# risc-mi/totalsegmentator2D

Hardware: AMD Instinct MI355X
Metric: 2-ch 512x512 slices/sec (higher is better)
Workload: dtype f32 storage/accumulate, products as 3x fp16-split MFMA (f16x3)

## Files before the change

### totalsegmentator2d_amd/csrc/dispatch.cpp

```cpp
#include "engine_internal.h"
#include "tile_dims.h"

#include <algorithm>

namespace ts2d {

namespace {

inline int lg_exact(int v) { return (v > 0 && (v & (v - 1)) == 0) ? ilog2(v) : -1; }

inline void tile_finish(TileGeom& g, int B, int Ht, int Wt, int sy, int sx, int taps) {
    const bool p2 = lg_exact(g.TH) >= 0 && lg_exact(g.TW) >= 0;
    g.lgTH = p2 ? ilog2(g.TH) : -1; g.lgTW = p2 ? ilog2(g.TW) : -1;
    if (g.NIMG > 1) { g.tiles_x = 1; g.tiles_y = 1; }
    else { g.tiles_x = (Wt + g.TW - 1) / g.TW; g.tiles_y = (Ht + g.TH - 1) / g.TH; }
    g.n_mtiles = (B + g.NIMG - 1) / g.NIMG * g.tiles_x * g.tiles_y;
    const int halo = (taps == 9) ? 3 : 1;
    g.PH = (g.TH - 1) * sy + halo; g.PW = (g.TW - 1) * sx + halo;
}

TileGeom tile_geom_pow2(int B, int Ht, int Wt, int sy, int sx, int taps) {
    TileGeom g{};
    g.TW = std::min(32, pow2ceil(Wt));
    g.TH = std::min(pow2ceil(Ht), kBM / g.TW);
// ... 208 lines not shown
        if (ck != K_NONE) {
            c.k = ck; c.fused_stats = true;
            if (ck == K_UP0 && f16) c.ppt = 4;
            c.bn = op.cout % 64 == 0 ? 64 : 32;
            if (Ht % 8 || Wt % 32) { bool ok = false; c.g = tile_geom_upc(B, Ht, Wt, ok); c.flex = true; }
            else c.g = tile_fixed(B, Ht, Wt, (ck == K_UPQ || ck == K_UPC_H2) ? 16 : 8, 32, 1, 1);
            if (ck == K_UPC_H || ck == K_UPC_H2) c.ks = e->ops[op.up_idx].cin % 64 == 0 ? 4 : 2;
            if (ck == K_UP0) {
                c.seg = segment_tiles(e, c.g);
                if (e->u0seg > 0 && (c.g.tiles_x * c.g.tiles_y) % e->u0seg == 0) c.seg = e->u0seg;
            }
            return c;
        }
    }
    c.bn = op.cout % 64 == 0 ? 64 : 32;
    if (!(op.split_ok && !exact)) {
        if (f16 && op.stride != 3) return c;
        c.k = K_EXACT;
        c.g = tile_geom(B, Ht, Wt, op.sy, op.sx, 9);
        c.fused_stats = c.g.NIMG == 1;
        return c;
    }
    const bool img32 = fits32((size_t)Hin * Win * std::max(op.cin, op.cin_skip) * 4) && fits32((size_t)Ht * Wt * op.cout * 4);
    if (op.stride == 2) {
        int s2k = 1;
        {
            const TileGeom g1 = tile_geom(B, Ht, Wt, 2, 2, 9);
            const int P1 = g1.PH * g1.PW * g1.NIMG;
            if (e->use_one && g1.NIMG == 1 && P1 <= 5 * kBlock && img32) s2k = fill_ksplit(e, (long long)g1.n_mtiles * (op.cout / c.bn), op.cin / 8, full);
        }
        if (s2k == 1 && op.s2v2_ok && e->use_s2v2 && e->use_one && Ht % 8 == 0 && Wt % 32 == 0 && img32 && magic_ok(tile_fixed(B, Ht, Wt, 8, 32, 2, 2))) {
            c.k = K_S2_V2; c.bn = op.bn2; c.fused_stats = true;
            c.g = tile_fixed(B, Ht, Wt, 8, 32, 2, 2);
            s2v2_variant(e, op, c);
            return c;
        }
        if (s2k == 1 && op.s2v2_ok && e->use_s2v2 && e->use_one && e->use_flex2 && img32 && (f16 || e->use_flex2 > 1)) {
            bool ok = false;
            const TileGeom gs = tile_geom_s2v2(B, Ht, Wt, ok);
            if (ok && magic_ok(gs)) { c.k = K_S2_V2; c.bn = op.bn2; c.fused_stats = true; c.flex = true; c.g = gs; s2v2_variant(e, op, c); return c; }
        }
        c.g = tile_geom(B, Ht, Wt, 2, 2, 9);
        c.ksplit = std::max(choose_ksplit(op, c.g), s2k);
        c.fused_stats = c.g.NIMG == 1 && c.ksplit == 1;
        const int P = c.g.PH * c.g.PW * c.g.NIMG;
        c.k = (e->use_one && c.g.NIMG == 1 && P <= 5 * kBlock && img32) ? K_S2_ONE : K_S2_GENERIC;
        return c;
    }
    if (op.res_ok && e->use_res && e->use_one && src.normed && op.skip < 0 && Ht % 8 == 0 && Wt % 32 == 0 && fits32((size_t)Ht * Wt * 32 * 4)) {
        c.k = (oi == 1 && fuse0_applies(e, H, W)) ? K_S1_RES32F : K_S1_RES32;
        c.fused_stats = true;
        c.g = tile_fixed(B, Ht, Wt, 8, 32, 1, 1);
        c.seg = segment_tiles(e, c.g);
        return c;
    }
    c.g = tile_geom(B, Ht, Wt, 1, 1, 9);
    c.ksplit = choose_ksplit(op, c.g);
    c.fused_stats = c.g.NIMG == 1;
    const int P = c.g.PH * c.g.PW * c.g.NIMG;
    const bool srcs_normed = src.normed && (op.skip < 0 || e->tensors[op.skip].normed);
    const bool tiles16 = Ht % 16 == 0 && Wt % 32 == 0 && c.g.NIMG == 1 && img32;
    if (c.g.NIMG == 1 && img32 && op.cout % c.bn == 0) {
        const bool can = f16 ? (op.h32_ok && P * 4 <= 6 * kBlock) : (e->use_one && P * 2 <= 3 * kBlock);
        const int sk = can ? fill_ksplit(e, (long long)c.g.n_mtiles * (op.cout / c.bn), ct / (f16 ? 32 : 16), full) : 1;
        if (sk > 1) {
            c.ksplit = sk; c.fused_stats = false;
            c.k = f16 ? K_S1_H32 : K_S1_ONE;
            return c;
        }
    }
    if (f16) {
        if (e->use_h2 && tiles16 && op.cout % 64 == 0 && op.skip < 0 && ct % 32 == 0 && src.normed && ct >= kH2Min) {
            c.k = K_S1_H2; c.bn = 64;
            c.g = tile_fixed(B, Ht, Wt, 16, 32, 1, 1);
            return c;
        }
        c.k = (op.h32_ok && c.g.NIMG == 1 && P * 4 <= 6 * kBlock && img32) ? K_S1_H32 : K_S1_GENERIC;
        return c;
    }
    const bool one = e->use_one && c.g.NIMG == 1 && P * 2 <= 3 * kBlock && img32;
    if (one && e->use_q && tiles16 && c.bn == 64 && ct >= 64 && srcs_normed && magic_ok(tile_fixed(B, Ht, Wt, 16, 32, 1, 1))) {
        c.k = K_S1_QP;
        c.g = tile_fixed(B, Ht, Wt, 16, 32, 1, 1);
        return c;
    }
    c.k = one ? K_S1_ONE : K_S1_GENERIC;
    return c;
}

const char* kernel_name(const Op& op, const Choice& c) {
    const bool b64 = c.bn == 64;
    switch (c.k) {
    case K_NONE: case K_FUSED_AWAY: return "";
    case K_FIRST: return c.first_split ? "conv3x3_first_split" : "conv3x3_first";
    case K_FIRST_STATS: return "conv3x3_first_stats";
    case K_EXACT: return op.type == OP_CONV ? "conv_mfma_f32" : "convT_mfma_f32";
    case K_S1_GENERIC: return "conv3x3_f16x3";
    case K_S1_ONE: return b64 ? "conv3x3_f16x3_one<64>" : "conv3x3_f16x3_one<32>";
    case K_S1_QP: return "conv3x3_f16x3_qp";
    case K_S1_H32: return b64 ? "conv3x3_h32<64>" : "conv3x3_h32<32>";
    case K_S1_H2: return "conv3x3_h2";
    case K_S1_RES32: return "conv3x3_res32";
    case K_S1_RES32F: return "conv3x3_res32f";
    case K_S2_V2: return c.bn == 128 ? (c.k32 ? "conv3x3s2_v2<128,k32>" : "conv3x3s2_v2<128>") : (c.k32 ? "conv3x3s2_v2<64,k32>" : "conv3x3s2_v2<64>");
    case K_S2_ONE: return "conv3x3s2_f16x3_one";
    case K_S2_GENERIC: return "conv3x3s2_f16x3";
// ... 157 lines not shown
```

### totalsegmentator2d_amd/csrc/engine.hip

```cpp
#include "engine_internal.h"
#include "kernels.h"
#include "kernels_f16x3.h"
#include "kernels_f16x3_convt.h"
#include "kernels_h32.h"
#include "kernels_head.h"
#include "kernels_f16x3_one.h"
#include "kernels_f16x3_qp.h"
#include "kernels_first.h"
#include "kernels_res32.h"
#include "kernels_s2v2.h"
#include "kernels_upc.h"
#include "kernels_up0.h"
#include "kernels_upq.h"
#include "kernels_upc_h.h"
#include "kernels_upc_h2.h"
#include "kernels_resblock.h"

#include <atomic>
#include <cstdio>
#include <cmath>
#include <cstdlib>
#include <cstring>
#include <string>
#include <type_traits>
// ... 205 lines not shown
int launch_composed(ts2d_engine* e, size_t oi, const Choice& c, const Run& r) {
    if (c.k == K_UP0) return launch_up0(e, oi, c, r);
    const Op& op = e->ops[oi]; const Op& up = e->ops[op.up_idx];
    const Tensor& xc = e->tensors[up.src]; const Tensor& sk = e->tensors[op.skip];
    const TileGeom& g = c.g;
    const float* wts = e->d_weights;
    const int bn = c.bn;
    UpcArgs ua{};
    ua.xc = xc.data; ua.scc = xc.scale; ua.shc = xc.shift; ua.Cb = up.cin;
    ua.xs = sk.data; ua.scs = sk.scale; ua.shs = sk.shift; ua.Cs = op.cin_skip;
    ua.wc = wts + op.dev_wc; ua.wk = wts + op.dev_wk; ua.bvar = wts + op.dev_bvar; ua.oscale = wts + op.dev_wcs;
    ua.dst = e->tensors[op.dst].data; ua.part = e->d_part;
    ua.B = r.B; ua.H = r.H >> op.ly; ua.W = r.W >> op.lx; ua.Cout = op.cout;
    ua.tiles_x = g.tiles_x; ua.tiles_y = g.tiles_y; ua.n_mtiles = g.n_mtiles; ua.n_ctiles = op.cout / bn;
    ua.TH = g.TH; ua.TW = g.TW; ua.inv_twc = 1.0f / (float)(g.TW / 2);
    ua.slope = e->arch.leaky_slope;
    ua.prof = prof_slots(e, oi); ua.dbg = e->dbg;
    const dim3 grid((ua.n_mtiles + 7) / 8 * 8 * ua.n_ctiles), block(kBlock);
    const bool b64 = bn == 64, flex = c.flex;
    hipError_t launch;
    if (c.k == K_UPC_H2) {
        launch = c.ks == 4 ? launch_max_lds<conv3x3_upc_h2<4>>(grid, block, kUh2Lds, r.st, ua) : launch_max_lds<conv3x3_upc_h2<2>>(grid, block, kUh2Lds, r.st, ua);
    } else if (c.k == K_UPC_H) {
        const size_t smem = std::max((size_t)c.ks * 2 * kUcPlane, (size_t)4 * kUsPlane + (size_t)2 * 9 * 2 * bn * 16);
        auto inst = [&](auto bn_, auto ks_) {
            constexpr int BN = decltype(bn_)::value, KS = decltype(ks_)::value;
            return flex ? launch_max_lds<conv3x3_upc_h<BN, KS, true>>(grid, block, smem, r.st, ua) : launch_max_lds<conv3x3_upc_h<BN, KS>>(grid, block, smem, r.st, ua);
        };
        using I32 = std::integral_constant<int, 32>; using I64 = std::integral_constant<int, 64>;
        using K2 = std::integral_constant<int, 2>; using K4 = std::integral_constant<int, 4>;
        launch = b64 ? (c.ks == 4 ? inst(I64{}, K4{}) : inst(I64{}, K2{})) : (c.ks == 4 ? inst(I32{}, K4{}) : inst(I32{}, K2{}));
    } else if (c.k == K_UPQ) {
        launch = launch_max_lds<conv3x3_upq>(grid, dim3(kUqThreads), kUqLds, r.st, ua);
    } else {
        const size_t smem = std::max((size_t)8 * kUcPlane, (size_t)4 * kUsPlane + (size_t)9 * 4 * bn * 16);
        if (b64) launch = flex ? launch_max_lds<conv3x3_upc<64, true>>(grid, block, smem, r.st, ua) : launch_max_lds<conv3x3_upc<64, false>>(grid, block, smem, r.st, ua);
        else launch = flex ? launch_max_lds<conv3x3_upc<32, true>>(grid, block, smem, r.st, ua) : launch_max_lds<conv3x3_upc<32, false>>(grid, block, smem, r.st, ua);
    }
    HIP_TRY(launch);
    return TS2D_OK;
}

int launch_res32(ts2d_engine* e, size_t oi, const Choice& c, const Run& r) {
    const Op& op = e->ops[oi];
    const Tensor& src = e->tensors[op.src];
    const float* wts = e->d_weights;
    Res32Args ra{};
    ra.src = src.data; ra.sc = src.scale; ra.sh = src.shift; ra.wres = wts + op.dev_wres; ra.bias = wts + op.dev_b;
    ra.oscale = wts + op.dev_ws; ra.dst = e->tensors[op.dst].data; ra.part = e->d_part;
    ra.B = r.B; ra.H = r.H >> op.ly; ra.W = r.W >> op.lx; ra.tiles_x = c.g.tiles_x; ra.tiles_y = c.g.tiles_y; ra.n_tiles = c.g.n_mtiles;
    ra.slope = e->arch.leaky_slope;
    ra.prof = prof_slots(e, oi);
    ra.seg = c.seg;
    const bool fuse0 = c.k == K_S1_RES32F;
    if (fuse0) {
        if (!e->fused_away[0]) return fail(TS2D_ERR_INVALID, "internal: fused second block without the statistics-only first pass");
        const Op& o0 = e->ops[0];
        ra.src = nullptr; ra.x0 = r.d_in; ra.C0 = o0.cin; ra.w0 = wts + o0.dev_wraw; ra.b0 = wts + o0.dev_b;
    }
    const dim3 grid(ra.n_tiles / ra.seg), block(kBlock);
    const hipError_t launch = with_storage(r.f16, [&](auto s) {
        using S = decltype(s); using ST = typename S::type;
        const size_t smem = S::np == 3 ? 9 * 2 * 4 * 512 + 8 * kResPS : 9 * 4 * 512 + 4 * kResPS + 1536;
        return fuse0 ? launch_max_lds<conv3x3_res32<ST, S::np, true>>(grid, block, smem, r.st, ra) : launch_max_lds<conv3x3_res32<ST, S::np, false>>(grid, block, smem, r.st, ra);
    });
    HIP_TRY(launch);
    return TS2D_OK;
}

int launch_head(ts2d_engine* e, size_t oi, const Choice& c, const Run& r) {
    const Op& op = e->ops[oi];
    const Tensor& src = e->tensors[op.src];
    const float* wts = e->d_weights;
    HeadArgs ha{};
    ha.src = src.data; ha.sc = src.scale; ha.sh = src.shift; ha.w = wts + op.dev_w; ha.bias = wts + op.dev_b;
    ha.logits = r.d_logits; ha.mask = r.d_mask; ha.C = src.C; ha.K = op.cout; ha.HW = r.H * r.W;
    ha.total = (long long)r.B * r.H * r.W; ha.slope = e->arch.leaky_slope; ha.nonfinite = e->d_flags;
    if (c.k == K_HEAD_MFMA) {
        ha.wph = wts + op.dev_wh; ha.oscale = wts + op.dev_ws;
        const int bpw = 16;
        const long long nblk = ha.total / 32;
        const dim3 grid((unsigned)((nblk + 4 * bpw - 1) / (4 * bpw)));
        const hipError_t launch = with_storage(r.f16, [&](auto s) { using S = decltype(s); return launch_kernel<head_mfma32<typename S::type, S::np>>(grid, dim3(256), 0, r.st, ha, bpw); });
        HIP_TRY(launch);
        return TS2D_OK;
    }
    const dim3 grid((unsigned)((ha.total + 255) / 256));
    const size_t smem = ((size_t)256 * (src.C + 1) + (size_t)op.cout * src.C + op.cout) * sizeof(float);
    const hipError_t launch = with_storage(r.f16, [&](auto s) {
        using ST = typename decltype(s)::type;
        return src.C == 32 ? launch_max_lds<head_1x1<32, ST>>(grid, dim3(256), smem, r.st, ha) : launch_max_lds<head_1x1<64, ST>>(grid, dim3(256), smem, r.st, ha);
    });
    HIP_TRY(launch);
    return TS2D_OK;
}

int launch_proj(ts2d_engine* e, size_t oi, const Choice& c, const Run& r) {
    const Op& op = e->ops[oi];
    const Tensor& src = e->tensors[op.src];
    ProjArgs pa{};
    pa.src = src.data; pa.sc = src.scale; pa.sh = src.shift; pa.w = e->d_weights + op.dev_w; pa.dst = e->tensors[op.dst].data;
    pa.part = c.fused_stats ? e->d_part : nullptr;
    pa.Cin = src.C; pa.Cout = op.cout; pa.sy = op.sy; pa.sx = op.sx;
    pa.Wt = r.W >> op.lx; pa.HW = (r.H >> op.ly) * pa.Wt; pa.Win = r.W >> src.lx; pa.M = r.B * pa.HW;
    pa.slope = e->arch.leaky_slope; pa.inv_n = 1.0f / (float)(op.sy * op.sx);
    if (!src.normed || src.linear || src.C % 32 || op.cout % c.bn || (r.H >> src.ly) != (r.H >> op.ly) * op.sy || pa.Win != pa.Wt * op.sx)
// ... 356 lines not shown
    if (he != hipSuccess) {
        rc = fail(he == hipErrorOutOfMemory ? TS2D_ERR_NOMEM : TS2D_ERR_HIP, "engine setup failed: %s", hipGetErrorString(he));
        ts2d_engine_destroy(e);
        return rc;
    }
    if (weights) {
        rc = upload_weights(e, weights, n_floats);
        if (rc != TS2D_OK) { ts2d_engine_destroy(e); return rc; }
    }
    *out = e;
    return TS2D_OK;
}

int ts2d_engine_create(const ts2d_arch_desc* arch, const float* weights, size_t n_floats, int device, ts2d_engine** out) {
    return create_engine("ts2d_engine_create", arch, nullptr, weights, n_floats, device, out);
}

int ts2d_engine_create_residual(const ts2d_arch_desc* arch, const ts2d_residual_desc* residual, const float* weights, size_t n_floats, int device,
                                ts2d_engine** out) {
    if (!residual) return fail(TS2D_ERR_INVALID, "ts2d_engine_create_residual: null argument");
    return create_engine("ts2d_engine_create_residual", arch, residual, weights, n_floats, device, out);
}

int ts2d_engine_load_weights(ts2d_engine* e, const float* weights, size_t n_floats) {
    if (!e || !weights) return fail(TS2D_ERR_INVALID, "ts2d_engine_load_weights: null argument");
    HIP_TRY(hipSetDevice(e->device));
    if (e->ws_busy) { HIP_TRY(hipEventSynchronize(e->ws_event)); e->ws_busy = false; }
    HIP_TRY(hipStreamSynchronize(e->stream));
    return upload_weights(e, weights, n_floats);
}

int ts2d_engine_weight_buffer(ts2d_engine* e, void** dev_ptr, size_t* n_bytes) {
    if (!e || !dev_ptr || !n_bytes) return fail(TS2D_ERR_INVALID, "ts2d_engine_weight_buffer: null argument");
    *dev_ptr = e->d_weights; *n_bytes = e->weight_floats * sizeof(float);
    return TS2D_OK;
}

int ts2d_engine_set_precision(ts2d_engine* e, int mode) {
    if (!e) return fail(TS2D_ERR_INVALID, "ts2d_engine_set_precision: null engine");
    if (mode != TS2D_PRECISION_F32_EXACT && mode != TS2D_PRECISION_F32_SPLIT_F16X3 && mode != TS2D_PRECISION_F16)
        return fail(TS2D_ERR_INVALID, "unknown precision mode %d", mode);
    if (mode == TS2D_PRECISION_F16 && e->residual)
        return fail(TS2D_ERR_INVALID, "TS2D_PRECISION_F16 is not supported on a residual-encoder engine (TS2D_PRECISION_F32_SPLIT_F16X3 and "
                    "TS2D_PRECISION_F32_EXACT are); the mode is unchanged");
    e->precision = mode;
    return TS2D_OK;
}

int ts2d_engine_set_option(ts2d_engine* e, const char* name, int value) {
    if (!e || !name) return fail(TS2D_ERR_INVALID, "ts2d_engine_set_option: null argument");
    struct B { const char* n; bool* p; };
    struct I { const char* n; int* p; int lo, hi; };
    const B bools[] = {{"one", &e->use_one}, {"s2v2", &e->use_s2v2}, {"q", &e->use_q}, {"h2", &e->use_h2},  {"uh2", &e->use_uh2},
                       {"first_split", &e->use_first_split}, {"sbk", &e->use_sbk}, {"s2k32", &e->use_s2k32}, {"up0", &e->use_up0}, {"upc", &e->use_upc}, {"res", &e->use_res}, {"fuse0", &e->use_fuse0}, {"flex", &e->use_flex}};
    const I ints[] = {{"u0seg", &e->u0seg, 0, 1 << 20}, {"flex2", &e->use_flex2, 0, 2}};
    bool found = false;
    for (const B& b : bools) if (!strcmp(name, b.n)) { *b.p = value != 0; found = true; }
    for (const I& i : ints) if (!strcmp(name, i.n)) {
        if (value < i.lo || value > i.hi) return fail(TS2D_ERR_INVALID, "option %s = %d out of range [%d, %d]", name, value, i.lo, i.hi);
        *i.p = value; found = true;
    }
    if (!found) return fail(TS2D_ERR_INVALID, "unknown option '%s' (one s2v2 q h2 uh2 up0 u0seg upc res fuse0 flex flex2 first_split sbk s2k32)", name);
    e->ws_precision = -1;
    ++e->opt_gen;
    return TS2D_OK;
}

int ts2d_engine_set_keep_activations(ts2d_engine* e, int enable) {
    if (!e) return fail(TS2D_ERR_INVALID, "ts2d_engine_set_keep_activations: null engine");
    e->keep_activations = enable != 0;
    return TS2D_OK;
}

int ts2d_engine_set_tile_dtype(ts2d_engine* e, int mode) {
    if (!e) return fail(TS2D_ERR_INVALID, "ts2d_engine_set_tile_dtype: null engine");
    if (mode != TS2D_TILE_F32 && mode != TS2D_TILE_F16) return fail(TS2D_ERR_INVALID, "unknown tile dtype %d", mode);
    e->tile_half = mode == TS2D_TILE_F16;
    return TS2D_OK;
}

int ts2d_engine_weights_ready(ts2d_engine* e) {
    if (!e) return fail(TS2D_ERR_INVALID, "ts2d_engine_weights_ready: null engine");
    e->weights_ready = true;
    return TS2D_OK;
}

int ts2d_engine_reserve(ts2d_engine* e, int B, int H, int W) {
    if (!e) return fail(TS2D_ERR_INVALID, "ts2d_engine_reserve: null engine");
    return reserve_checked(e, B, H, W, kBySize);
}

int ts2d_engine_workspace_bytes(ts2d_engine* e, int B, int H, int W, size_t* n_bytes) {
    if (!e || !n_bytes) return fail(TS2D_ERR_INVALID, "ts2d_engine_workspace_bytes: null argument");
    const int divy = 1 << e->lvl_y[e->arch.n_stages - 1], divx = 1 << e->lvl_x[e->arch.n_stages - 1];
    if (B < 1 || H < divy || W < divx || H % divy || W % divx)
        return fail(TS2D_ERR_INVALID, "shape B=%d H=%d W=%d: H and W must be positive multiples of %d and %d", B, H, W, divy, divx);
    *n_bytes = workspace_layout(e, B, H, W, kBySize).bytes;
    return TS2D_OK;
}

int ts2d_engine_set_workspace(ts2d_engine* e, void* dev_ptr, size_t n_bytes) {
    if (!e) return fail(TS2D_ERR_INVALID, "ts2d_engine_set_workspace: null engine");
    if (dev_ptr && (reinterpret_cast<uintptr_t>(dev_ptr) & 255)) return fail(TS2D_ERR_INVALID, "ts2d_engine_set_workspace: the pointer must be 256-byte aligned");
    HIP_TRY(hipSetDevice(e->device));
    if (e->ws_busy) { HIP_TRY(hipEventSynchronize(e->ws_event)); e->ws_busy = false; }
    HIP_TRY(hipStreamSynchronize(e->stream));
    if (e->d_ws && !e->ws_external) HIP_TRY(hipFree(e->d_ws));
    e->d_ws = reinterpret_cast<char*>(dev_ptr); e->ws_bytes = dev_ptr ? n_bytes : 0; e->ws_external = dev_ptr != nullptr;
    e->ws_precision = -1; e->wsB = 0;
    for (Tensor& t : e->tensors) { t.data = nullptr; t.bytes = 0; t.resident = false; }
    e->lastB = 0;
    return TS2D_OK;
}

int ts2d_engine_forward(ts2d_engine* e, const float* input, int B, int H, int W, float* logits, uint32_t* mask_packed,
// ... 213 lines not shown
```

### totalsegmentator2d_amd/csrc/engine_internal.h

```cpp
#pragma once
#include "../../include/ts2d_engine.h"
#include <hip/hip_runtime_api.h>
#include "device_tables.h"

#include <atomic>
#include <cstddef>
#include <cstdint>
#include <string>
#include <vector>

#pragma GCC visibility push(hidden)
namespace ts2d {

int fail(int code, const char* fmt, ...) __attribute__((format(printf, 2, 3)));
const char* last_error();

#define HIP_TRY(expr)                                                                                     \
    do {                                                                                                  \
        hipError_t _e = (expr);                                                                           \
        if (_e != hipSuccess)                                                                             \
            return fail(_e == hipErrorOutOfMemory ? TS2D_ERR_NOMEM : TS2D_ERR_HIP, "%s failed: %s (%s:%d)", \
                        #expr, hipGetErrorString(_e), __FILE__, __LINE__);                                \
    } while (0)
#define TRY(expr) do { int _rc = (expr); if (_rc != TS2D_OK) return _rc; } while (0)
// ... 80 lines not shown
    int bn = 0;
    int ksplit = 1;
    bool fused_stats = false;
    int ppt = 1;
    bool first_full = false;
    bool flex = false;
    bool first_split = false;
    bool k32 = false;
    int npp = 0, nch = 0;
    int seg = 0;
    int ks = 0;
    const char* name = "";
};

inline int pow2ceil(int v) { int p = 1; while (p < v) p <<= 1; return p; }
inline int ilog2(int v) { int l = 0; while ((1 << l) < v) ++l; return l; }
inline int ct_total(const Op& op) { return op.cin + op.cin_skip; }

}

#pragma GCC visibility pop

struct ts2d_engine {
    ts2d_arch_desc arch{};
    int lvl_y[TS2D_MAX_STAGES] = {0}, lvl_x[TS2D_MAX_STAGES] = {0};
    int device = 0;
    int cin_pad = 8;
    std::vector<ts2d::Tensor> tensors;
    std::vector<ts2d::Op> ops;
    size_t blob_floats = 0;
    ts2d_arch_desc user_arch{};
    bool residual = false;
    int n_blocks[TS2D_MAX_STAGES] = {0};
    bool padded = false;
    size_t user_blob_floats = 0;
    float* d_weights = nullptr; size_t weight_floats = 0;
    bool weights_ready = false;
    int precision = TS2D_PRECISION_F32_SPLIT_F16X3;
    int num_cus = 256;
    int tile_half = 0;
    int tiled_inf = 0;
    bool use_one = true;
    bool use_s2v2 = true;
    bool use_q = true;
    bool use_h2 = true;
    bool use_uh2 = true;
    bool use_s2k32 = true;
    bool use_sbk = true;
    bool use_first_split = true;
    bool use_up0 = true;
    int u0seg = 0;
    bool use_upc = true;
    bool use_res = true;
    bool use_fuse0 = true;
    bool diagnosing = false;
    int use_flex2 = 2;
    bool use_flex = true;
    int dbg = 0;
    unsigned long long* d_prof = nullptr;
    std::vector<char> fused_away;
    char* d_ws = nullptr; size_t ws_bytes = 0; int wsB = 0, wsH = 0, wsW = 0;
    bool ws_external = false;
    uint32_t ws_token = 0;
    std::vector<ts2d::Choice> plan; int planB = 0, planH = 0, planW = 0, plan_prec = -1; unsigned plan_gen = 0, opt_gen = 1; bool plan_full = false;
    char* d_stage = nullptr; size_t stage_bytes = 0;
    bool ws_full = false;
    bool last_full = false;
    int ws_precision = -1; bool ws_keep = false;
    bool keep_activations = false;
    float* d_part = nullptr;
    float* d_partial = nullptr;
    float* d_up = nullptr;
    float* d_in_stage = nullptr; float* d_logit_stage = nullptr; uint32_t* d_mask_stage = nullptr;
    hipStream_t stream = nullptr;
    bool profiling = false;
    std::vector<ts2d::Launch> launches; size_t n_launched = 0;
    int lastB = 0, lastH = 0, lastW = 0; hipStream_t last_stream = nullptr; bool last_f16 = false;
    char* d_sw = nullptr; size_t sw_bytes = 0;
    hipEvent_t ws_event = nullptr; hipStream_t ws_stream = nullptr; bool ws_busy = false;
    int* d_flags = nullptr;
    bool checked_input = false; const float* last_input = nullptr;
};

#pragma GCC visibility push(hidden)
namespace ts2d {

ts2d_arch_desc pad_arch(const ts2d_arch_desc& a, bool& padded);
void expand_blob(const ts2d_arch_desc& ua, const ts2d_arch_desc& pa, const int* n_blocks, const float* ub, std::vector<float>& pb);
int build_program(ts2d_engine* e);
int tensor_index(ts2d_engine* e, const std::string& name);

void pack_weights(const ts2d_engine* e, const float* blob, float* out);
float f16_to_f32(uint16_t hb);

constexpr size_t kSbkElems = (size_t)2 * 256 * 256 * 64;
constexpr bool kBySize = false, kFullBatch = true;

Choice choose(const ts2d_engine* e, size_t oi, int B, int H, int W, bool full);
std::vector<Choice> choose_all(const ts2d_engine* e, int B, int H, int W, bool full);
const std::vector<Choice>& planned(ts2d_engine* e, int B, int H, int W, bool full);

struct ActPlan { std::vector<size_t> off, size; std::vector<char> used, reused; size_t bytes = 0; };
struct WsLayout {
    ActPlan plan; std::vector<size_t> o_sc, o_sh; size_t o_part = 0, o_pk = 0, o_up = 0, bytes = 0;
    bool has_up = false;
};
// ... 40 lines not shown
```

### totalsegmentator2d_amd/csrc/kernels_res32.h

```cpp
#pragma once
#include "kernels_f16x3.h"
#include "kernels_h32.h"

namespace ts2d {

struct Res32Args {
    const void* src; const float* sc; const float* sh;
    const void* wres;
    const float* bias;
    const float* oscale;
    void* dst;
    float* part;
    int B, H, W;
    int tiles_x, tiles_y;
    int n_tiles;
    int seg;
    float slope;
    unsigned long long* prof;
    const float* x0; int C0;
    const float* w0; const float* b0;
};

constexpr int kResPW = 34, kResP = 340, kResPS = 352 * 16;

template <typename ST, int NP, bool FUSE = false>
__global__ __launch_bounds__(kBlock, 2) void conv3x3_res32(const Res32Args a) {
    constexpr int NPP = NP == 3 ? 2 : 1;
    constexpr int WB = 9 * NPP * 4 * 512;
    constexpr int NL = sizeof(ST) == 4 ? 2 : 1;
    constexpr int NU = 6;
    extern __shared__ __attribute__((aligned(16))) unsigned char smem8[];
    typedef unsigned u32x4 __attribute__((ext_vector_type(4)));

    const int tid = threadIdx.x, lane = tid & 63;
    const int w = __builtin_amdgcn_readfirstlane(tid >> 6);
    const int r = lane & 31, h = lane >> 5;

    const int tpi = a.tiles_x * a.tiles_y;
    const int t0 = (int)blockIdx.x * a.seg;
    if (t0 >= a.n_tiles) return;
    const int t1 = t0 + a.seg;
    const int n = t0 / tpi;
    int trem = t0 - n * tpi;
    int txi = trem / a.tiles_y, tyi = trem - txi * a.tiles_y;

    {
        const uint4* wsrc = reinterpret_cast<const uint4*>(a.wres);
#pragma unroll
        for (int k = 0; k < (WB / 16 + kBlock - 1) / kBlock; ++k) {
            const int sl = tid + k * kBlock;
            if (sl < WB / 16) *reinterpret_cast<uint4*>(smem8 + sl * 16) = wsrc[NPP == 2 ? sl : (sl >> 7) * 256 + (sl & 127)];
        }
    }
    unsigned char* sP = smem8 + WB;
    const int sg = (lane >> 3) & 3, pl = (lane & 7) + 8 * (lane >> 5);
    auto scratch32 = [&](int ww, int half) -> float* {
        if (NPP == 2) return reinterpret_cast<float*>(sP + (2 * ww + half) * kResPS + kResP * 16);
        return reinterpret_cast<float*>(sP + NPP * 4 * kResPS + (ww * 2 + half) * 192);
    };
    unsigned rel[FUSE ? 1 : NU];
    unsigned emask = 0;
    bool last_unit = false;
    const int swr = sg * kResPS + (16 * w + pl) * 16;
    const size_t img_bytes = (size_t)a.H * a.W * 32 * sizeof(ST);
    u32x4 pv[FUSE ? 1 : NU][NL];
    const int r2 = lane & 31, h2 = lane >> 5;
    constexpr int NK = 3;
    unsigned xrel[FUSE ? NK : 1], pq[FUSE ? NK : 1];
    float xv[FUSE ? NK : 1][FUSE ? 9 : 1];
    float wr0[FUSE ? 9 : 1], scq[FUSE ? 16 : 1], shq[FUSE ? 16 : 1];
    float bq[(FUSE && sizeof(ST) != 4) ? 16 : 1];
    typedef unsigned u32x4w __attribute__((ext_vector_type(4)));
    u32x4w wsp[FUSE ? 4 : 1];
    float inv_s0 = 1.f;
    const bool have3 = w != 3;
    __amdgpu_buffer_rsrc_t rs, rsx;
    if constexpr (!FUSE) {
#pragma unroll
        for (int it = 0; it < NU; ++it) {
            const int p = 64 * it + 16 * w + pl;
            const int py = p / kResPW, px = p - py * kResPW;
            rel[it] = (unsigned)(((py * a.W + px) * 32 + 8 * sg) * (int)sizeof(ST));
            if (p < kResP) emask |= ((py == 0 ? 1u : 0u) | (py == 9 ? 2u : 0u) | (px == 0 ? 4u : 0u) | (px == kResPW - 1 ? 8u : 0u)) << (4 * it);
        }
        last_unit = 64 * (NU - 1) + 16 * w + pl < kResP;
        rs = __builtin_amdgcn_make_buffer_rsrc(const_cast<unsigned char*>(reinterpret_cast<const unsigned char*>(a.src)) + (size_t)n * img_bytes,
                                               0, (int)img_bytes, 0x00020000);
    } else {
#pragma unroll
        for (int k = 0; k < NK; ++k) {
            const int p = 32 * (w + 4 * k) + r2;
            const int py = p / kResPW, px = p - py * kResPW;
            xrel[k] = (unsigned)(((h2 * a.H + py) * a.W + px) * 4);
            pq[k] = (unsigned)((py << 8) | px);
            if (p < kResP) emask |= ((py == 0 ? 1u : 0u) | (py == 9 ? 2u : 0u) | (px == 0 ? 4u : 0u) | (px == kResPW - 1 ? 8u : 0u)) << (4 * k);
        }
        const size_t in_bytes = (size_t)a.C0 * a.H * a.W * 4;
        rsx = __builtin_amdgcn_make_buffer_rsrc(const_cast<float*>(a.x0) + (size_t)n * a.C0 * a.H * a.W, 0, (int)in_bytes, 0x00020000);
#pragma unroll
        for (int tap = 0; tap < 9; ++tap) wr0[tap] = h2 < a.C0 ? a.w0[((size_t)r2 * a.C0 + h2) * 9 + tap] : 0.f;
        {
            float wmax = 0.f;
#pragma unroll
            for (int tap = 0; tap < 9; ++tap) wmax = fmaxf(wmax, fabsf(wr0[tap]));
#pragma unroll
            for (int d = 1; d < 64; d *= 2) wmax = fmaxf(wmax, __shfl_xor(wmax, d));
            int e2 = 0;
            (void)frexpf(wmax, &e2);
            const bool sane = wmax > 0.f && wmax < 3.0e38f;
            const float S0 = sane ? ldexpf(1.f, 12 - e2) : 1.f;
            inv_s0 = sane ? ldexpf(1.f, e2 - 12) : 1.f;
            unsigned short wh[9], wl[9];
#pragma unroll
            for (int tap = 0; tap < 9; ++tap) {
                wr0[tap] *= S0;
                const _Float16 hh = (_Float16)wr0[tap], ll = (_Float16)(wr0[tap] - (float)hh);
                wh[tap] = __builtin_bit_cast(unsigned short, hh); wl[tap] = __builtin_bit_cast(unsigned short, ll);
            }
            auto pk = [](unsigned short lo_, unsigned short hi_) { return (unsigned)lo_ | ((unsigned)hi_ << 16); };
            wsp[0] = u32x4w{pk(wh[0], wh[1]), pk(wh[2], wh[3]), pk(wh[0], wh[1]), pk(wh[2], wh[3])};
            wsp[1] = u32x4w{pk(wh[4], wh[5]), pk(wh[6], wh[7]), pk(wh[4], wh[5]), pk(wh[6], wh[7])};
            wsp[2] = u32x4w{pk(wh[8], wh[8]), pk(wl[8], 0), 0u, 0u};
            wsp[3] = u32x4w{pk(wl[0], wl[1]), pk(wl[2], wl[3]), pk(wl[4], wl[5]), pk(wl[6], wl[7])};
        }
#pragma unroll
        for (int i = 0; i < 16; ++i) {
            const int c = (i & 3) + 8 * (i >> 2) + 4 * h2;
            const float s_ = a.sc[(size_t)n * 32 + c], t_ = a.sh[(size_t)n * 32 + c], b_ = a.b0[c];
            if constexpr (sizeof(ST) == 4) { scq[i] = s_ * inv_s0; shq[i] = __builtin_fmaf(b_, s_, t_); }
            else { scq[i] = s_; shq[i] = t_; bq[i] = b_; }
        }
    }
    auto prefetch = [&](int ptx, int pty) {
        if constexpr (!FUSE) {
            const unsigned org = (unsigned)((((pty * 8 - 1) * a.W + (ptx * 32 - 1)) * 32) * (int)sizeof(ST));
#pragma unroll
            for (int it = 0; it < NU; ++it)
#pragma unroll
                for (int l = 0; l < NL; ++l)
                    pv[it][l] = __builtin_amdgcn_raw_buffer_load_b128(rs, org + rel[it] + 16 * l, 0, 0);
        } else {
            const int oy0 = pty * 8 - 2, ox0 = ptx * 32 - 2;
            const bool pe = (pty == 0) | (pty == a.tiles_y - 1) | (ptx == 0) | (ptx == a.tiles_x - 1);
            const unsigned org = (unsigned)((oy0 * a.W + ox0) * 4);
#pragma unroll
            for (int k = 0; k < NK; ++k) {
                if (k < NK - 1 || have3) {
#pragma unroll
                    for (int tap = 0; tap < 9; ++tap) {
                        const int dy = tap / 3, dx = tap - 3 * dy;
                        unsigned vo = org + xrel[k];
                        unsigned so = (unsigned)((dy * a.W + dx) * 4);
                        if (pe) {
                            const int iy = oy0 + (int)(pq[k] >> 8) + dy, ix = ox0 + (int)(pq[k] & 255u) + dx;
                            const bool ok = ((unsigned)iy < (unsigned)a.H) & ((unsigned)ix < (unsigned)a.W) & (h2 < a.C0);
                            vo = ok ? vo + so : 0x80000000u;
                            so = 0;
                        }
                        xv[k][tap] = __builtin_bit_cast(float, __builtin_amdgcn_raw_buffer_load_b32(rsx, vo, so, 0));
                    }
                }
            }
        }
    };
    prefetch(txi, tyi);

    const int wb32 = h * 512 + r * 16;
    const int pb32 = WB + h * kResPS + (2 * w * kResPW + r) * 16;
    const float bv32 = a.bias[r];
    const float oscale = *a.oscale;
    const _Float16 slope_h = (_Float16)a.slope;
    const unsigned slope2 = (unsigned)__builtin_bit_cast(unsigned short, slope_h) * 0x10001u;
    const auto rsd = __builtin_amdgcn_make_buffer_rsrc(reinterpret_cast<unsigned char*>(a.dst) + (size_t)n * img_bytes, 0, (int)img_bytes, 0x00020000);
    const float* ps = a.sc + (size_t)n * 32 + 8 * sg; const float* pt = a.sh + (size_t)n * 32 + 8 * sg;
    f32x4 nsa, nsb, nta, ntb;
    if constexpr (!FUSE) {
        nsa = *reinterpret_cast<const f32x4*>(ps); nsb = *reinterpret_cast<const f32x4*>(ps + 4);
        nta = *reinterpret_cast<const f32x4*>(pt); ntb = *reinterpret_cast<const f32x4*>(pt + 4);
    }
    const f32x4 slope4 = f32x4{a.slope, a.slope, a.slope, a.slope};

    TS2D_PROF_DECL(a.prof);
    for (int t = t0; t < t1; ++t) {
        const unsigned edge = (tyi == 0 ? 1u : 0u) | (tyi == a.tiles_y - 1 ? 2u : 0u) | (txi == 0 ? 4u : 0u) | (txi == a.tiles_x - 1 ? 8u : 0u);
        if constexpr (!FUSE) {
#pragma unroll
        for (int it = 0; it < NU; ++it) {
            if (it < NU - 1 || last_unit) {
                unsigned char* d = sP + swr + it * 1024;
                if constexpr (sizeof(ST) == 4) {
                    f32x4 va = __builtin_bit_cast(f32x4, pv[it][0]), vb = __builtin_bit_cast(f32x4, pv[it][NL - 1]);
                    va = va * nsa + nta; vb = vb * nsb + ntb;
                    const f32x4 na = va * slope4, nb2 = vb * slope4;
#pragma unroll
                    for (int e = 0; e < 4; ++e) { va[e] = fmaxf(va[e], na[e]); vb[e] = fmaxf(vb[e], nb2[e]); }
                    uint4 hi, lo;
                    split_hi_lo_8(va, vb, hi, lo);
                    *reinterpret_cast<uint4*>(d) = hi;
                    if (NPP == 2) *reinterpret_cast<uint4*>(d + 4 * kResPS) = lo;
                } else {
                    uint4 x = uint4{pv[it][0][0], pv[it][0][1], pv[it][0][2], pv[it][0][3]};
                    *reinterpret_cast<uint4*>(d) = norm_lrelu_8(x, nsa, nsb, nta, ntb, slope2);
                }
            }
        }
        if (edge) {
            const unsigned hit = emask & (edge * 0x111111u);
#pragma unroll
            for (int it = 0; it < NU; ++it)
                if (hit & (0xFu << (4 * it))) {
                    unsigned char* d = sP + swr + it * 1024;
                    *reinterpret_cast<uint4*>(d) = uint4{0u, 0u, 0u, 0u};
                    if (NPP == 2) *reinterpret_cast<uint4*>(d + 4 * kResPS) = uint4{0u, 0u, 0u, 0u};
                }
        }
        } else {
        const unsigned hit = edge ? (emask & (edge * 0x111u)) : 0u;
#pragma unroll
        for (int k = 0; k < NK; ++k) {
            if (k < NK - 1 || have3) {
                f32x16 acc0 = kZero16;
                float amax = 0.f;
#pragma unroll
                for (int tap = 0; tap < 9; tap += 3) amax = fmaxf(amax, fmaxf(fabsf(xv[k][tap]), fmaxf(fabsf(xv[k][tap + 1]), fabsf(xv[k][tap + 2]))));
                if (__builtin_amdgcn_ballot_w64(!(amax < 65504.f)) == 0) {
                    uint4 xh, xl;
                    split_hi_lo_8(f32x4{xv[k][0], xv[k][1], xv[k][2], xv[k][3]}, f32x4{xv[k][4], xv[k][5], xv[k][6], xv[k][7]}, xh, xl);
                    const _Float16 h8 = (_Float16)xv[k][8], l8 = (_Float16)(xv[k][8] - (float)h8);
                    const unsigned uh8 = __builtin_bit_cast(unsigned short, h8), ul8 = __builtin_bit_cast(unsigned short, l8);
                    const u32x4w xb0 = u32x4w{xh.x, xh.y, xl.x, xl.y}, xb1 = u32x4w{xh.z, xh.w, xl.z, xl.w};
                    const u32x4w xb2 = u32x4w{uh8 | (ul8 << 16), uh8, 0u, 0u}, xb3 = u32x4w{xh.x, xh.y, xh.z, xh.w};
                    acc0 = __builtin_amdgcn_mfma_f32_32x32x16_f16(__builtin_bit_cast(half8, wsp[0]), __builtin_bit_cast(half8, xb0), acc0, 0, 0, 0);
                    acc0 = __builtin_amdgcn_mfma_f32_32x32x16_f16(__builtin_bit_cast(half8, wsp[1]), __builtin_bit_cast(half8, xb1), acc0, 0, 0, 0);
                    acc0 = __builtin_amdgcn_mfma_f32_32x32x16_f16(__builtin_bit_cast(half8, wsp[2]), __builtin_bit_cast(half8, xb2), acc0, 0, 0, 0);
                    acc0 = __builtin_amdgcn_mfma_f32_32x32x16_f16(__builtin_bit_cast(half8, wsp[3]), __builtin_bit_cast(half8, xb3), acc0, 0, 0, 0);
                } else {
#pragma unroll
                    for (int tap = 0; tap < 9; ++tap) acc0 = __builtin_amdgcn_mfma_f32_32x32x2f32(wr0[tap], xv[k][tap], acc0, 0, 0, 0);
                }
                const bool zero = (hit >> (4 * k)) & 0xFu;
                const int p = 32 * (w + 4 * k) + r2;
                unsigned char* d = sP + p * 16 + 8 * h2;
                typedef unsigned u32x2 __attribute__((ext_vector_type(2)));
                if constexpr (sizeof(ST) == 4) {
                    float v[16];
#pragma unroll
                    for (int i = 0; i < 16; ++i) { const float y = __builtin_fmaf(acc0[i], scq[i], shq[i]); v[i] = fmaxf(y, y * a.slope); }
#pragma unroll
                    for (int qq = 0; qq < 2; ++qq) {
                        uint4 hi, lo;
                        split_hi_lo_8(f32x4{v[8 * qq], v[8 * qq + 1], v[8 * qq + 2], v[8 * qq + 3]},
                                      f32x4{v[8 * qq + 4], v[8 * qq + 5], v[8 * qq + 6], v[8 * qq + 7]}, hi, lo);
                        if (zero) { hi = uint4{0u, 0u, 0u, 0u}; lo = hi; }
                        if (k < NK - 1 || p < kResP) {
                            *reinterpret_cast<u32x2*>(d + (2 * qq) * kResPS) = u32x2{hi.x, hi.y};
                            *reinterpret_cast<u32x2*>(d + (2 * qq + 1) * kResPS) = u32x2{hi.z, hi.w};
                            *reinterpret_cast<u32x2*>(d + (2 * qq + 4) * kResPS) = u32x2{lo.x, lo.y};
                            *reinterpret_cast<u32x2*>(d + (2 * qq + 5) * kResPS) = u32x2{lo.z, lo.w};
                        }
                    }
                } else {
                    typedef _Float16 half4 __attribute__((ext_vector_type(4)));
#pragma unroll
                    for (int q = 0; q < 4; ++q) {
                        half4 o;
#pragma unroll
                        for (int e = 0; e < 4; ++e) {
                            const int i = 4 * q + e;
                            const float raw = (float)(_Float16)__builtin_fmaf(acc0[i], inv_s0, bq[i]);
                            const _Float16 y = (_Float16)__builtin_fmaf(raw, scq[i], shq[i]);
                            const _Float16 ng = y * slope_h;
                            o[e] = zero ? (_Float16)0.f : (y > ng ? y : ng);
                        }
                        if (k < NK - 1 || p < kResP) *reinterpret_cast<half4*>(d + q * kResPS) = o;
                    }
                }
            }
        }
        }
        TS2D_STAMP_AT(a.prof, 0)
        lds_barrier();
        TS2D_STAMP_AT(a.prof, 1)

        int ntx = txi, nty = tyi + 1;
        if (nty == a.tiles_y) { nty = 0; ntx = txi + 1; }
        if (t + 1 < t1) prefetch(ntx, nty);

        f32x16 acc[2];
#pragma unroll
        for (int mt = 0; mt < 2; ++mt)
#pragma unroll
            for (int i = 0; i < 16; ++i) acc[mt][i] = 0.f;
        __builtin_amdgcn_s_setprio(1);
        half8 fw[2][2][NPP], fx[2][2][2][NPP];
#define TS2D_R32_LOAD(SET, TAP) { constexpr int dy_ = (TAP) / 3, dx_ = (TAP) - 3 * dy_; \
            _Pragma("unroll") for (int ks = 0; ks < 2; ++ks) _Pragma("unroll") for (int pt2 = 0; pt2 < NPP; ++pt2) { \
                fw[SET][ks][pt2] = *reinterpret_cast<const half8*>(smem8 + wb32 + (((TAP) * NPP + pt2) * 4 + 2 * ks) * 512); \
                _Pragma("unroll") for (int mt = 0; mt < 2; ++mt) \
                    fx[SET][mt][ks][pt2] = *reinterpret_cast<const half8*>(smem8 + pb32 + (pt2 * 4 + 2 * ks) * kResPS + ((mt + dy_) * kResPW + dx_) * 16); } }
#define TS2D_R32_TAP(TAP) { constexpr int c_ = (TAP) & 1; \
            if constexpr ((TAP) + 1 < 9) TS2D_R32_LOAD(c_ ^ 1, (TAP) + 1) \
            if constexpr (NP == 3) { \
                _Pragma("unroll") for (int ks = 0; ks < 2; ++ks) _Pragma("unroll") for (int mt = 0; mt < 2; ++mt) \
                    acc[mt] = __builtin_amdgcn_mfma_f32_32x32x16_f16(fx[c_][mt][ks][NPP - 1], fw[c_][ks][0], acc[mt], 0, 0, 0); \
                _Pragma("unroll") for (int ks = 0; ks < 2; ++ks) _Pragma("unroll") for (int mt = 0; mt < 2; ++mt) \
                    acc[mt] = __builtin_amdgcn_mfma_f32_32x32x16_f16(fx[c_][mt][ks][0], fw[c_][ks][NPP - 1], acc[mt], 0, 0, 0); } \
            _Pragma("unroll") for (int ks = 0; ks < 2; ++ks) _Pragma("unroll") for (int mt = 0; mt < 2; ++mt) \
                acc[mt] = __builtin_amdgcn_mfma_f32_32x32x16_f16(fx[c_][mt][ks][0], fw[c_][ks][0], acc[mt], 0, 0, 0); \
            __builtin_amdgcn_sched_barrier(0); }
        TS2D_R32_LOAD(0, 0)
        TS2D_R32_TAP(0) TS2D_R32_TAP(1) TS2D_R32_TAP(2) TS2D_R32_TAP(3) TS2D_R32_TAP(4) TS2D_R32_TAP(5) TS2D_R32_TAP(6) TS2D_R32_TAP(7) TS2D_R32_TAP(8)
#undef TS2D_R32_TAP
#undef TS2D_R32_LOAD
        __builtin_amdgcn_s_setprio(0);
        TS2D_STAMP_AT(a.prof, 2)

        {
            const float kv = stat_pivot(round_act<ST>(__builtin_fmaf(acc[0][0], oscale, bv32)));
            float s = 0.f, q = 0.f;
#pragma unroll
            for (int mt = 0; mt < 2; ++mt) {
                const unsigned voff = (unsigned)(((((tyi * 8 + 2 * w + mt) * a.W + txi * 32 + 4 * h) * 32) + r) * (int)sizeof(ST));
#pragma unroll
                for (int i = 0; i < 16; ++i) {
                    const float v = __builtin_fmaf(acc[mt][i], oscale, bv32);
                    buffer_store_act<ST>(v, rsd, voff + (unsigned)((((i & 3) + 8 * (i >> 2)) * 32) * (int)sizeof(ST)), 0);
                    const float d = round_act<ST>(v) - kv;
                    s += d; q = __builtin_fmaf(d, d, q);
                }
            }
            s += __shfl_xor(s, 32); q += __shfl_xor(q, 32);
            if (h == 0) { float* sc = scratch32(w, r >> 4) + (r & 15); sc[0] = s; sc[16] = q; sc[32] = kv; }
        }
        TS2D_STAMP_AT(a.prof, 3)
        lds_barrier();
        if (FUSE ? (tid >= 192 && tid < 224) : tid < 32) {
            const int co = tid & 31, c = co & 15;
            const float* s0 = scratch32(0, co >> 4);
            f32x4 acc4 = f32x4{s0[c], s0[16 + c], s0[32 + c], 64.f};
#pragma unroll
            for (int ww = 1; ww < 4; ++ww) {
                const float* sw_ = scratch32(ww, co >> 4);
                const float d = sw_[32 + c] - acc4[2];
                acc4[1] += sw_[16 + c] + d * (2.f * sw_[c] + 64.f * d);
                acc4[0] += sw_[c] + 64.f * d;
                acc4[3] += 64.f;
            }
            *reinterpret_cast<f32x4*>(a.part + (((size_t)n * tpi + (t - n * tpi)) * 32 + co) * 4) = acc4;
        }
        txi = ntx; tyi = nty;
        TS2D_STAMP_AT(a.prof, 4)
    }
    TS2D_PROF_FLUSH(a.prof)
}

}
```

Baseline: 2955.

## Reuse vertical halo rows across consecutive tiles via LDS ring buffer in res32 conv

```diff
diff --git a/totalsegmentator2d_amd/csrc/dispatch.cpp b/totalsegmentator2d_amd/csrc/dispatch.cpp
--- a/totalsegmentator2d_amd/csrc/dispatch.cpp
+++ b/totalsegmentator2d_amd/csrc/dispatch.cpp
@@ -284,6 +284,7 @@
         c.fused_stats = true;
         c.g = tile_fixed(B, Ht, Wt, 8, 32, 1, 1);
         c.seg = segment_tiles(e, c.g);
+        if (e->u0seg > 0 && (c.g.tiles_x * c.g.tiles_y) % e->u0seg == 0) c.seg = e->u0seg;
         return c;
     }
     c.g = tile_geom(B, Ht, Wt, 1, 1, 9);
diff --git a/totalsegmentator2d_amd/csrc/engine.hip b/totalsegmentator2d_amd/csrc/engine.hip
--- a/totalsegmentator2d_amd/csrc/engine.hip
+++ b/totalsegmentator2d_amd/csrc/engine.hip
@@ -281,6 +281,7 @@
     ra.slope = e->arch.leaky_slope;
     ra.prof = prof_slots(e, oi);
     ra.seg = c.seg;
+    ra.halo = e->use_halo ? 1 : 0;
     const bool fuse0 = c.k == K_S1_RES32F;
     if (fuse0) {
         if (!e->fused_away[0]) return fail(TS2D_ERR_INVALID, "internal: fused second block without the statistics-only first pass");
@@ -743,7 +744,7 @@
     struct B { const char* n; bool* p; };
     struct I { const char* n; int* p; int lo, hi; };
     const B bools[] = {{"one", &e->use_one}, {"s2v2", &e->use_s2v2}, {"q", &e->use_q}, {"h2", &e->use_h2},  {"uh2", &e->use_uh2},
-                       {"first_split", &e->use_first_split}, {"sbk", &e->use_sbk}, {"s2k32", &e->use_s2k32}, {"up0", &e->use_up0}, {"upc", &e->use_upc}, {"res", &e->use_res}, {"fuse0", &e->use_fuse0}, {"flex", &e->use_flex}};
+                       {"first_split", &e->use_first_split}, {"sbk", &e->use_sbk}, {"s2k32", &e->use_s2k32}, {"up0", &e->use_up0}, {"upc", &e->use_upc}, {"res", &e->use_res}, {"fuse0", &e->use_fuse0}, {"halo", &e->use_halo}, {"flex", &e->use_flex}};
     const I ints[] = {{"u0seg", &e->u0seg, 0, 1 << 20}, {"flex2", &e->use_flex2, 0, 2}};
     bool found = false;
     for (const B& b : bools) if (!strcmp(name, b.n)) { *b.p = value != 0; found = true; }
@@ -751,7 +752,7 @@
         if (value < i.lo || value > i.hi) return fail(TS2D_ERR_INVALID, "option %s = %d out of range [%d, %d]", name, value, i.lo, i.hi);
         *i.p = value; found = true;
     }
-    if (!found) return fail(TS2D_ERR_INVALID, "unknown option '%s' (one s2v2 q h2 uh2 up0 u0seg upc res fuse0 flex flex2 first_split sbk s2k32)", name);
+    if (!found) return fail(TS2D_ERR_INVALID, "unknown option '%s' (one s2v2 q h2 uh2 up0 u0seg upc res fuse0 halo flex flex2 first_split sbk s2k32)", name);
     e->ws_precision = -1;
     ++e->opt_gen;
     return TS2D_OK;
diff --git a/totalsegmentator2d_amd/csrc/engine_internal.h b/totalsegmentator2d_amd/csrc/engine_internal.h
--- a/totalsegmentator2d_amd/csrc/engine_internal.h
+++ b/totalsegmentator2d_amd/csrc/engine_internal.h
@@ -156,6 +156,7 @@
     int u0seg = 0;
     bool use_upc = true;
     bool use_res = true;
+    bool use_halo = true;
     bool use_fuse0 = true;
     bool diagnosing = false;
     int use_flex2 = 2;
diff --git a/totalsegmentator2d_amd/csrc/kernels_res32.h b/totalsegmentator2d_amd/csrc/kernels_res32.h
--- a/totalsegmentator2d_amd/csrc/kernels_res32.h
+++ b/totalsegmentator2d_amd/csrc/kernels_res32.h
@@ -19,9 +19,12 @@
     unsigned long long* prof;
     const float* x0; int C0;
     const float* w0; const float* b0;
+    int halo;
 };
 
+
 constexpr int kResPW = 34, kResP = 340, kResPS = 352 * 16;
+constexpr int kResRow = kResPW * 16;
 
 template <typename ST, int NP, bool FUSE = false>
 __global__ __launch_bounds__(kBlock, 2) void conv3x3_res32(const Res32Args a) {
@@ -38,6 +41,7 @@
 
     const int tpi = a.tiles_x * a.tiles_y;
     const int t0 = (int)blockIdx.x * a.seg;
+    const bool ring = !FUSE && a.halo != 0;
     if (t0 >= a.n_tiles) return;
     const int t1 = t0 + a.seg;
     const int n = t0 / tpi;
@@ -61,7 +65,9 @@
     unsigned rel[FUSE ? 1 : NU];
     unsigned emask = 0;
     bool last_unit = false;
-    const int swr = sg * kResPS + (16 * w + pl) * 16;
+    const int swr = sg * kResPS;
+    const unsigned swp = (unsigned)((16 * w + pl) * 16);
+    auto ring_slot = [](unsigned o) { return o < o - 10u * kResRow ? o : o - 10u * kResRow; };
     const size_t img_bytes = (size_t)a.H * a.W * 32 * sizeof(ST);
     u32x4 pv[FUSE ? 1 : NU][NL];
     const int r2 = lane & 31, h2 = lane >> 5;
@@ -131,14 +137,16 @@
             else { scq[i] = s_; shq[i] = t_; bq[i] = b_; }
         }
     }
-    auto prefetch = [&](int ptx, int pty) {
+    auto prefetch = [&](int ptx, int pty, bool keep) {
         if constexpr (!FUSE) {
             const unsigned org = (unsigned)((((pty * 8 - 1) * a.W + (ptx * 32 - 1)) * 32) * (int)sizeof(ST));
 #pragma unroll
-            for (int it = 0; it < NU; ++it)
+            for (int it = 0; it < NU; ++it) {
+                if (it == 0 && keep) continue;
 #pragma unroll
                 for (int l = 0; l < NL; ++l)
                     pv[it][l] = __builtin_amdgcn_raw_buffer_load_b128(rs, org + rel[it] + 16 * l, 0, 0);
+            }
         } else {
             const int oy0 = pty * 8 - 2, ox0 = ptx * 32 - 2;
             const bool pe = (pty == 0) | (pty == a.tiles_y - 1) | (ptx == 0) | (ptx == a.tiles_x - 1);
@@ -163,10 +171,10 @@
             }
         }
     };
-    prefetch(txi, tyi);
+    prefetch(txi, tyi, false);
 
     const int wb32 = h * 512 + r * 16;
-    const int pb32 = WB + h * kResPS + (2 * w * kResPW + r) * 16;
+    const int pb32 = WB + h * kResPS + r * 16;
     const float bv32 = a.bias[r];
     const float oscale = *a.oscale;
     const _Float16 slope_h = (_Float16)a.slope;
@@ -180,14 +188,18 @@
     }
     const f32x4 slope4 = f32x4{a.slope, a.slope, a.slope, a.slope};
 
+    int rb = 0;
+    bool keep = false;
     TS2D_PROF_DECL(a.prof);
     for (int t = t0; t < t1; ++t) {
+        const unsigned swt = swp + (unsigned)(rb * kResRow);
         const unsigned edge = (tyi == 0 ? 1u : 0u) | (tyi == a.tiles_y - 1 ? 2u : 0u) | (txi == 0 ? 4u : 0u) | (txi == a.tiles_x - 1 ? 8u : 0u);
         if constexpr (!FUSE) {
 #pragma unroll
         for (int it = 0; it < NU; ++it) {
+            if (it == 0 && keep) continue;
             if (it < NU - 1 || last_unit) {
-                unsigned char* d = sP + swr + it * 1024;
+                unsigned char* d = sP + swr + ring_slot(swt + it * 1024);
                 if constexpr (sizeof(ST) == 4) {
                     f32x4 va = __builtin_bit_cast(f32x4, pv[it][0]), vb = __builtin_bit_cast(f32x4, pv[it][NL - 1]);
                     va = va * nsa + nta; vb = vb * nsb + ntb;
@@ -205,11 +217,11 @@
             }
         }
         if (edge) {
-            const unsigned hit = emask & (edge * 0x111111u);
+            const unsigned hit = emask & (edge * 0x111111u) & (keep ? ~0xFu : ~0u);
 #pragma unroll
             for (int it = 0; it < NU; ++it)
                 if (hit & (0xFu << (4 * it))) {
-                    unsigned char* d = sP + swr + it * 1024;
+                    unsigned char* d = sP + swr + ring_slot(swt + it * 1024);
                     *reinterpret_cast<uint4*>(d) = uint4{0u, 0u, 0u, 0u};
                     if (NPP == 2) *reinterpret_cast<uint4*>(d + 4 * kResPS) = uint4{0u, 0u, 0u, 0u};
                 }
@@ -284,7 +296,11 @@
 
         int ntx = txi, nty = tyi + 1;
         if (nty == a.tiles_y) { nty = 0; ntx = txi + 1; }
-        if (t + 1 < t1) prefetch(ntx, nty);
+        const bool nkeep = ring && nty != 0;
+        if (t + 1 < t1) prefetch(ntx, nty, nkeep);
+        int sa = rb + 2 * w, sb = rb + 2 * w + 2;
+        sa = sa >= 10 ? sa - 10 : sa; sb = sb >= 10 ? sb - 10 : sb;
+        const int pbA = pb32 + sa * kResRow, pbB = pb32 + (sb - 2) * kResRow;
 
         f32x16 acc[2];
 #pragma unroll
@@ -297,7 +313,7 @@
             _Pragma("unroll") for (int ks = 0; ks < 2; ++ks) _Pragma("unroll") for (int pt2 = 0; pt2 < NPP; ++pt2) { \
                 fw[SET][ks][pt2] = *reinterpret_cast<const half8*>(smem8 + wb32 + (((TAP) * NPP + pt2) * 4 + 2 * ks) * 512); \
                 _Pragma("unroll") for (int mt = 0; mt < 2; ++mt) \
-                    fx[SET][mt][ks][pt2] = *reinterpret_cast<const half8*>(smem8 + pb32 + (pt2 * 4 + 2 * ks) * kResPS + ((mt + dy_) * kResPW + dx_) * 16); } }
+                    fx[SET][mt][ks][pt2] = *reinterpret_cast<const half8*>(smem8 + (mt + dy_ < 2 ? pbA : pbB) + (pt2 * 4 + 2 * ks) * kResPS + ((mt + dy_) * kResPW + dx_) * 16); } }
 #define TS2D_R32_TAP(TAP) { constexpr int c_ = (TAP) & 1; \
             if constexpr ((TAP) + 1 < 9) TS2D_R32_LOAD(c_ ^ 1, (TAP) + 1) \
             if constexpr (NP == 3) { \
@@ -349,6 +365,8 @@
             *reinterpret_cast<f32x4*>(a.part + (((size_t)n * tpi + (t - n * tpi)) * 32 + co) * 4) = acc4;
         }
         txi = ntx; tyi = nty;
+        keep = nkeep;
+        rb = nkeep ? (rb >= 2 ? rb - 2 : rb + 8) : 0;
         TS2D_STAMP_AT(a.prof, 4)
     }
     TS2D_PROF_FLUSH(a.prof)
```

Measured after the change: 2954. No clear change (-0.0%).
